# weibohuang0314/pixel_aware_gyro_aided_klt_feature_tracker

Measured on AMD Instinct MI355X. Metric: tracked features/sec (21x21, 3-lvl, 30 iter), higher is better.
Workload: dtype f32 sampling, f64 normal equations; 1 GPU; cfg1_euroc_752x480: 752x480 pair, 1000 keypoints (1000/GPU), gyro-predicted affine init, h=10, L=3, I=30 (synthetic stand-in for BASELINE configs[1]); mode=shard-weak, features_total=1000, features_active=1000, step_mode=graph

## Files before the change

### __graft_entry__.py

```python
from __future__ import annotations

import os
import subprocess
import sys

ROOT = os.path.dirname(os.path.abspath(__file__))
PKG = os.path.join(ROOT, "pixel_aware_gyro_aided_klt_feature_tracker_amd")
CSRC = os.path.join(PKG, "csrc")
HIP_LIB = os.path.join(PKG, "libpagk_hip.so")
HOST_LIB = os.path.join(PKG, "libpagk_tracker.so")

HIPCC_FLAGS = [
    "--offload-arch=gfx950", "-O3", "-std=c++17", "-fPIC", "-shared",
    "-ffp-contract=off", "-fno-fast-math",
    "-Wall", "-Wno-unused-function",
]


def _newer(target: str, sources: list[str]) -> bool:
    if not os.path.exists(target):
        return False
    t = os.path.getmtime(target)
    return all(os.path.getmtime(s) <= t for s in sources)


def _run(cmd: list[str]) -> str:
    r = subprocess.run(cmd, capture_output=True, text=True)
    if r.returncode != 0:
        sys.stderr.write(r.stdout + r.stderr)
        raise RuntimeError("build failed: " + " ".join(cmd))
    return r.stderr


RESOURCES_JSON = os.path.join(PKG, "kernel_resources.json")

RESOURCE_CLAIMS = {
    "k_track_blockILi2ELi25ELi4ELb0ELb0ELb1": (128, 0, 4),
    "k_track_blockILi1ELi25ELi4ELb0ELb0ELb1": (96, 0, 4),
    "k_track_quadILi7ELb1": (128, 44, 4),
    "k_track_blockILi2ELi25ELi4ELb0ELb0ELb0": (128, 20, 4),
    "k_track_blockILi1ELi25ELi4ELb0ELb0ELb0": (128, 6, 4),
    "k_track_quadILi7ELb0": (128, 48, 4),
    "k_track_block_pyrILi2ELi25ELb0": (128, 24, 4),
    "k_track_resume_liveILi2ELi25ELb0": (128, 64, 4),
    "k_track_resumeILi2ELi25ELb0": (128, 64, 4),
    "k_track_resume_liveILi2ELi25ELb1": (128, 48, 4),
    "k_track_resumeILi2ELi25ELb1": (128, 48, 4),
    "k_track_block_pyrILi2ELi25ELb1": (128, 8, 4),
    "k_track_block5ILi2ELi25ELb1": (96, 16, 5),
    "k_rectifyILi1ELb1": (64, 0, 8),
    "k_rectifyILi3ELb1": (64, 0, 8),
    "k_rectifyILi4ELb1": (64, 0, 8),
}


RESOURCE_CLAIMS_ALL_VARIANTS = {
    "k_track_blockILi4ELi25ELi2ELb1ELb0ELb1": (128, 10, 4),
    "k_track_blockILi4ELi25ELi2ELb1ELb0ELb0": (128, 32, 4),
    "k_track_rowsILi7": (128, 64, 4),
}


def _parse_resource_remarks(text: str) -> dict:
    import re
    out, cur = {}, None
    keys = {"VGPRs": "vgprs", "AGPRs": "agprs", "ScratchSize [bytes/lane]": "scratch_bytes_per_lane",
            "Occupancy [waves/SIMD]": "waves_per_simd", "VGPRs Spill": "vgpr_spills", "SGPRs Spill": "sgpr_spills",
            "TotalSGPRs": "sgprs"}
    for line in text.splitlines():
        m = re.search(r"remark:\s+Function Name: (\S+)", line)
        if m:
            cur = out.setdefault(m.group(1), {})
            continue
        m = re.search(r"remark:\s+([A-Za-z \[\]/]+): (\d+)", line)
        if m and cur is not None and m.group(1).strip() in keys:
            cur[keys[m.group(1).strip()]] = int(m.group(2))
    return out


def _parse_resources_from_asm(text: str) -> dict:
    import re
    out, cur, fn = {}, None, None
    keys = {".vgpr_count": "vgprs", ".agpr_count": "agprs", ".private_segment_fixed_size": "scratch_bytes_per_lane",
            ".vgpr_spill_count": "vgpr_spills", ".sgpr_spill_count": "sgpr_spills", ".sgpr_count": "sgprs",
            ".group_segment_fixed_size": "lds_bytes"}
    occ = {}
    for line in text.splitlines():
        m = re.match(r"^(_Z\w+):", line)
        if m:
            fn = m.group(1)
            continue
        m = re.match(r"^; Occupancy: (\d+)", line)
        if m and fn:
            occ[fn] = int(m.group(1))
            continue
        if line.startswith("  - .agpr_count:") or line.startswith("  - .args:"):
            cur = {}
        m = re.match(r"^\s+(?:- )?(\.[a-z_]+):\s+(\S+)\s*$", line)
        if m and cur is not None:
            if m.group(1) == ".name":
                out[m.group(2)] = cur
            elif m.group(1) in keys and m.group(2).isdigit():
                cur[keys[m.group(1)]] = int(m.group(2))
    for k, v in out.items():
        v["waves_per_simd"] = occ.get(k, 0)
        for f in ("vgprs", "agprs", "scratch_bytes_per_lane", "vgpr_spills", "sgpr_spills", "sgprs"):
            v.setdefault(f, 0)
    return {k: v for k, v in out.items() if "vgprs" in v}


def check_resources(res: dict, claims: dict | None = None) -> None:
    bad = []
    for key, (max_vgpr, max_spill, min_occ) in (claims or RESOURCE_CLAIMS).items():
        hits = [v for k, v in res.items() if key in k]
        if not hits:
            bad.append(f"kernel {key} is missing from the code object")
        for v in hits:
            if v["vgprs"] > max_vgpr or v["vgpr_spills"] > max_spill or v["waves_per_simd"] < min_occ:
                bad.append(f"{key}: {v} violates the documented allocation (<= {max_vgpr} VGPRs, <= {max_spill} "
                           f"spilled, >= {min_occ} waves/SIMD)")
    if bad:
        raise RuntimeError("; ".join(bad))


PRIORITY_CLAIMS = {
    "k_track_blockILi2ELi25ELi4ELb0ELb0ELb1": (3, 2, 1, 0),
    "k_track_blockILi2ELi25ELi4ELb0ELb0ELb0": (3, 2, 1, 0),
    "k_track_block5ILi2ELi25ELb1": (3, 2, 0),
}


def check_priorities(asm_text: str, claims: dict | None = None) -> list[str]:
    import re
    body, fn = {}, None
    for line in asm_text.splitlines():
# ... 129 lines not shown
```

### pixel_aware_gyro_aided_klt_feature_tracker_amd/csrc/pagk_hip.hip

```cpp
#include <hip/hip_runtime.h>

#include <algorithm>
#include <array>
#include <cmath>
#include <cstdio>
#include <cstdlib>
#include <cstring>
#include <new>
#include <utility>
#include <vector>

#include "../../include/pagk.h"
#include "pagk_kernels.h"
#include "pagk_layout.h"
#include "pagk_select.h"

using namespace pagk;

namespace {

constexpr int kSlots = 6;
constexpr int kUserSlots = 4;

struct DevBuf {
// ... 21 lines not shown
    int device = 0;
    hipStream_t own_stream = nullptr;
    hipStream_t stream = nullptr;
    FrameSlot slots[kSlots];
    enum Buf {
        FEAT,
        SCORE,
        FIT,
        FITIO,
        HAND,
        HANDIO,
        DET,
        FAST,
        RECT_ENTRIES,
        RECT_STAGE,
        QUAD_WS,
        SUSP,
        LV,
        kBufs
    };
    DevBuf buf[kBufs];
    int fit_n = 0, fit_iters = 0;
    int rect_w = 0, rect_h = 0, rect_wp = 0;
    void *queue = nullptr;
    int quad_capacity[PAGK_MAX_HALF_PATCH + 1] = {};
    int rows_capacity[PAGK_MAX_HALF_PATCH + 1] = {};
    int rows_waves_cap = 0;
    int *susp_count_dev = nullptr;
    struct BatchDesc {
        void *host = nullptr, *dev = nullptr;
        hipEvent_t used = nullptr;
        bool recorded = false;
    };
    static constexpr int kBatchRing = 6, kBatchPerCapture = 4, kBatchMaxStreams = 64;
    BatchDesc batch_ring[kBatchRing];
    int batch_turn = 0;
    bool batch_seen = false;
    std::vector<BatchDesc> cap_batch;
    int cap_batch_used = 0;
    hipEvent_t ev_batch = nullptr;
    int *lv_error = nullptr;
    int *lv_error_dev = nullptr;
    hipStream_t aux_stream = nullptr;
    hipEvent_t ev_fork = nullptr, ev_join = nullptr;
    int susp_lone = 1;
    int finisher_wgs = 16;
    int finisher_polls = 20000;
    int level_polls = 300000;
    int quad_budget = -1;
    int cus = 0;
    bool capturing = false;
    static constexpr int kGraphs = 8;
    hipGraph_t graphs[kGraphs] = {};
    hipGraphExec_t graph_execs[kGraphs] = {};
    struct GraphSeg {
        enum Kind { GRAPH, FINISHER, JOIN } kind = GRAPH;
        hipGraph_t g = nullptr;
        hipGraphExec_t ex = nullptr;
        const void *fn = nullptr;
        TrackArgs args;
        int grid = 0;
        size_t lds = 0;
    };
    std::vector<GraphSeg> pre_segs[kGraphs];
    std::vector<BatchDesc> graph_batch[kGraphs];
    std::vector<GraphSeg> cap_segs;
    hipEvent_t ev_trk[2] = {}, ev_pyr[2] = {};
    bool trk_timed = false, pyr_timed = false;
    int kernel = 0;
    bool last_handover = false;
    int concurrency = 1;
    int last_variant = -1;
    int mfma_min_features = 0x7fffffff;
    int wave_min_features = 6000;
    int quad_min_features = 7000;
    int block5_min_features = 2500;
    int prio_k = 4;
    unsigned long long *prio_stats = nullptr;
    bool block5_window = true;
    int levels_min_features = 6000;
    int levels_shift = 0;
    bool levels_shared = false;
    bool unfused_pyramid = false;
    char err[256] = {0};
};

namespace {

#define HIPCHK(ctx, call)                                                                              \
    do {                                                                                               \
        hipError_t e_ = (call);                                                                        \
        if (e_ != hipSuccess) {                                                                        \
            snprintf((ctx)->err, sizeof((ctx)->err), "%s:%d %s -> %s", __FILE__, __LINE__, #call,     \
                     hipGetErrorString(e_));                                                           \
            return e_ == hipErrorOutOfMemory ? PAGK_E_NOMEM : PAGK_E_HIP;                              \
        }                                                                                              \
    } while (0)

#define NOT_WHILE_CAPTURING(ctx, what)                                                                 \
    do {                                                                                               \
        if ((ctx)->capturing) {                                                                        \
            snprintf((ctx)->err, sizeof((ctx)->err), "%s is not capturable: use the *_device entry points between pagk_graph_begin and pagk_graph_end", what); \
            return PAGK_E_ARG;                                                                         \
        }                                                                                              \
    } while (0)

int level_dims(int w, int h, int L, int *lw, int *lh)
{
    lw[0] = w;
    lh[0] = h;
    for (int l = 1; l < L; l++) {
        lw[l] = (int)(lw[l - 1] * 0.5);
        lh[l] = (int)(lh[l - 1] * 0.5);
        if (lw[l] < 1 || lh[l] < 1) return PAGK_E_ARG;
    }
    return PAGK_OK;
}

bool in_capture(pagk_ctx *ctx)
{
    if (ctx->capturing) return true;
    hipStreamCaptureStatus st = hipStreamCaptureStatusNone;
    return hipStreamIsCapturing(ctx->stream, &st) != hipSuccess || st != hipStreamCaptureStatusNone;
}

int no_live_graphs(pagk_ctx *ctx, const char *what, const char *hint)
{
    for (int k = 0; k < pagk_ctx::kGraphs; k++)
        if (ctx->graph_execs[k]) {
            snprintf(ctx->err, sizeof(ctx->err), "%s would have to grow while graph %d of this context is alive (its nodes hold the old "
                     "pointers): destroy the graph first, or %s", what, k, hint);
            return PAGK_E_ARG;
        }
    return PAGK_OK;
}

enum GrowPolicy {
    GROW_FREELY = 0,
    NOT_IN_CAPTURE = 1,
    NOT_UNDER_GRAPH = 2,
    NOT_IN_CAPTURE_NOR_UNDER_GRAPH = NOT_IN_CAPTURE | NOT_UNDER_GRAPH,
};

int release(pagk_ctx *ctx, DevBuf &b)
{
    if (b.ptr) HIPCHK(ctx, hipFree(b.ptr));
    if (b.host) HIPCHK(ctx, hipHostFree(b.host));
    b.ptr = b.host = nullptr;
    b.bytes = 0;
    return PAGK_OK;
}

int reserve(pagk_ctx *ctx, DevBuf &b, size_t bytes, GrowPolicy policy, const char *what, const char *hint = "")
{
    if (bytes <= b.bytes) return PAGK_OK;
    if ((policy & NOT_IN_CAPTURE) && in_capture(ctx)) {
        snprintf(ctx->err, sizeof(ctx->err), "%s would have to grow inside a graph capture: %s", what, hint);
        return PAGK_E_ARG;
    }
    int rc = (policy & NOT_UNDER_GRAPH) ? no_live_graphs(ctx, what, hint) : PAGK_OK;
    if (rc || (rc = release(ctx, b))) return rc;
    HIPCHK(ctx, hipMalloc(&b.ptr, bytes));
    if (b.mirrored) HIPCHK(ctx, hipHostMalloc(&b.host, bytes, hipHostMallocDefault));
    b.bytes = bytes;
    return PAGK_OK;
}
// ... 66 lines not shown
            return nullptr;
        }
        return &lead->cap_batch[lead->cap_batch_used++];
    }
    pagk_ctx::BatchDesc *desc = &lead->batch_ring[lead->batch_turn];
    lead->batch_turn = (lead->batch_turn + 1) % pagk_ctx::kBatchRing;
    if (!desc->dev) {
        if ((*rc = batch_desc_alloc(lead, *desc)) != PAGK_OK) {
            batch_desc_free(*desc);
            return nullptr;
        }
    } else if (desc->recorded) {
        if (hipEventSynchronize(desc->used) != hipSuccess) {
            snprintf(lead->err, sizeof(lead->err), "hipEventSynchronize of a batch descriptor's last user failed");
            *rc = PAGK_E_HIP;
            return nullptr;
        }
    }
    lead->batch_seen = true;
    return desc;
}
int batch_desc_used(pagk_ctx *lead, pagk_ctx::BatchDesc *desc)
{
    if (in_capture(lead)) return PAGK_OK;
    HIPCHK(lead, hipEventRecord(desc->used, lead->stream));
    desc->recorded = true;
    return PAGK_OK;
}

int slot_alloc(pagk_ctx *ctx, FrameSlot &s, const int *lw, const int *lh, int L, GrowPolicy policy)
{
    size_t sizes[2 * kMaxLevels];
    for (int l = 0; l < L; l++) {
        sizes[l] = (size_t)lw[l] * lh[l];
        sizes[L + l] = sizes[l] * 4;
    }
    const Layout<2 * kMaxLevels> lay(sizes, 2 * L);
    int rc = reserve(ctx, s.block, lay.total, policy, "the frame slot", "run the same calls once before pagk_graph_begin");
    if (rc) return rc;
    for (int l = 0; l < L; l++) {
        s.u8[l] = lay.at<uint8_t>(s.block.ptr, l);
        s.quad[l] = lay.at<uint32_t>(s.block.ptr, L + l);
    }
    s.w = lw[0];
    s.h = lh[0];
    s.L = L;
    return PAGK_OK;
}

int slot_reserve(pagk_ctx *ctx, FrameSlot &s, int w, int h, int L)
{
    int lw[kMaxLevels], lh[kMaxLevels];
    int rc = level_dims(w, h, L, lw, lh);
    return rc ? rc : slot_alloc(ctx, s, lw, lh, L, NOT_IN_CAPTURE);
}

int make_pyr_args(const FrameSlot &s, const uint8_t *src0, int64_t pitch0, int wrap0, PyrArgs *out)
{
    int lw[kMaxLevels], lh[kMaxLevels];
    level_dims(s.w, s.h, s.L, lw, lh);
    PyrArgs pa;
    memset(&pa, 0, sizeof pa);
    pa.src = src0;
    pa.pitch = pitch0;
    pa.wrap0 = wrap0;
    pa.n_levels = s.L;
    int nb = 0;
    for (int l = 0; l < 4; l++) {
        pa.first_block[l] = nb;
        if (l < s.L) {
            pa.cols[l] = lw[l];
            pa.rows[l] = lh[l];
            pa.u8[l] = s.u8[l];
            pa.quad[l] = s.quad[l];
            nb += (lw[l] * lh[l] + 255) / 256;
        }
    }
    pa.first_block[4] = nb;
    for (int l = s.L; l < 4; l++) pa.first_block[l] = nb;
    *out = pa;
    return nb;
}

bool pyramid_fusable(const FrameSlot &s)
{
    int lw[kMaxLevels], lh[kMaxLevels];
    level_dims(s.w, s.h, s.L, lw, lh);
    bool all_even = s.L <= 4;
    for (int l = 0; l + 1 < s.L; l++) all_even = all_even && !(lw[l] & 1) && !(lh[l] & 1);
    return all_even;
}

int slot_build(pagk_ctx *ctx, FrameSlot &s, const uint8_t *src0, int64_t pitch0, int wrap0)
{
    s.pad0 = wrap0 ? 0 : 2;
    s.img0 = src0, s.pitch0 = pitch0;
    int lw[kMaxLevels], lh[kMaxLevels];
    level_dims(s.w, s.h, s.L, lw, lh);
    dim3 blk(32, 8);
    if (ctx->ev_pyr[0] && !in_capture(ctx)) HIPCHK(ctx, hipEventRecord(ctx->ev_pyr[0], ctx->stream));
    bool all_even = true;
    for (int l = 0; l + 1 < s.L; l++) all_even = all_even && !(lw[l] & 1) && !(lh[l] & 1);
    if (s.L <= 4 && !ctx->unfused_pyramid && all_even) {
        PyrArgs pa;
        const int nb = make_pyr_args(s, src0, pitch0, wrap0, &pa);
        hipLaunchKernelGGL(k_pyramid_fused, dim3(nb), dim3(256), 0, ctx->stream, pa);
        HIPCHK(ctx, hipGetLastError());
        if (ctx->ev_pyr[1] && !in_capture(ctx)) HIPCHK(ctx, hipEventRecord(ctx->ev_pyr[1], ctx->stream));
        if (!in_capture(ctx)) ctx->pyr_timed = true;
        s.wrap0 = wrap0;
        s.valid = true;
        return PAGK_OK;
    }
    const uint8_t *src = src0;
    int64_t pitch = pitch0;
    for (int l = 0; l < s.L; l++) {
        if (l > 0) {
            dim3 grd((lw[l] + 31) / 32, (lh[l] + 7) / 8);
            if (!(lw[l - 1] & 1) && !(lh[l - 1] & 1))
                hipLaunchKernelGGL(k_pyr_down, grd, blk, 0, ctx->stream, src, pitch, lw[l], lh[l], s.u8[l]);
            else
                hipLaunchKernelGGL(k_pyr_down_linear, grd, blk, 0, ctx->stream, src, pitch, lw[l - 1], lh[l - 1], lw[l],
                                   lh[l], 1. / ((double)lw[l] / lw[l - 1]), 1. / ((double)lh[l] / lh[l - 1]), s.u8[l]);
            src = s.u8[l];
            pitch = lw[l];
        }
        dim3 grd((lw[l] + 31) / 32, (lh[l] + 7) / 8);
        hipLaunchKernelGGL(k_build_quads, grd, blk, 0, ctx->stream, src, pitch, lw[l], lh[l], l == 0 ? wrap0 : 1,
                           s.quad[l]);
    }
    HIPCHK(ctx, hipGetLastError());
    if (ctx->ev_pyr[1] && !in_capture(ctx)) HIPCHK(ctx, hipEventRecord(ctx->ev_pyr[1], ctx->stream));
    if (!in_capture(ctx)) ctx->pyr_timed = true;
    s.wrap0 = wrap0;
    s.valid = true;
    return PAGK_OK;
}

int check_params(const pagk_params *p)
{
    if (!p) return PAGK_E_ARG;
    if (p->half_patch < 1 || p->half_patch > PAGK_MAX_HALF_PATCH) return PAGK_E_ARG;
    if (p->iterations < 0 || p->pyramids < 1 || p->pyramids > PAGK_MAX_PYRAMIDS) return PAGK_E_ARG;
    if (p->inverse) return PAGK_E_UNSUPPORTED;
    if (p->solver_variant & ~(SV_LOWER_SEQ | SV_UPPER_TREE | SV_NORM_SEQ | SV_LLT_RECIP | SV_PIVOT_TREE)) return PAGK_E_ARG;
    return PAGK_OK;
}

void fill_level(DevLevel &d, const FrameSlot &s, int l)
{
    int w = s.w, h = s.h;
    for (int k = 0; k < l; k++) {
        w = (int)(w * 0.5);
        h = (int)(h * 0.5);
    }
    d.quad = s.quad[l];
    d.cols = w;
    d.rows = h;
    d.fcols = (float)w;
    d.frows = (float)h;
    d.fcols_m1 = (float)(w - 1);
    d.frows_m1 = (float)(h - 1);
}

int lv_check(pagk_ctx *ctx)
{
    if (ctx->lv_error && *static_cast<volatile int *>(ctx->lv_error) != 0) {
        *static_cast<volatile int *>(ctx->lv_error) = 0;
        snprintf(ctx->err, sizeof(ctx->err), "a wave of a tracking launch gave up waiting (for the level above, or for the other chain wave's sums)");
        return PAGK_E_HIP;
    }
    return PAGK_OK;
}

using TrackFn = void (*)(TrackArgs);
struct TrackKernels {
    TrackFn block[2] = {}, block5 = nullptr;
    void (*block_pyr[2])(TrackArgs, PyrArgs) = {};
    TrackFn resume[2] = {}, resume_live[2] = {};
    TrackFn wave[2] = {};
    TrackFn quad[2] = {}, levels[2] = {}, batch[2] = {};
    TrackFn relaxed = nullptr;
    TrackFn mfma[2] = {}, rows = nullptr;
};

template <int H>
constexpr TrackKernels track_kernels()
{
    constexpr PatchShape s = patch_shape(H);
// ... 416 lines not shown
        case PAGK_E_ARG: return "invalid argument";
        case PAGK_E_HIP: return "HIP runtime error";
        case PAGK_E_NOMEM: return "out of memory";
        case PAGK_E_UNSUPPORTED: return "unsupported mode";
        case PAGK_E_NODEVICE: return "no HIP device";
        case PAGK_E_NCCL: return "RCCL error";
        case PAGK_E_CAPACITY: return "output capacity too small";
        default: return "unknown error";
    }
}

const char *pagk_last_error(const pagk_ctx *ctx) { return ctx ? ctx->err : ""; }

void pagk_params_default(pagk_params *p)
{
    if (!p) return;
    memset(p, 0, sizeof *p);
    p->half_patch = 5;
    p->iterations = 10;
    p->pyramids = 3;
    p->has_gyro_predict_initial = 1;
    p->inverse = 0;
    p->consider_illumination = 1;
    p->consider_affine = 1;
    p->regularization_penalty = 0;
    p->calculate_ncc = 0;
    p->lambda = 1.0f;
    p->alpha = 0.5f;
    p->max_distance = 25;
    p->inv_log_max_dist = 0.0f;
    p->fx = p->fy = 1.0f;
    p->n_dist_coef = 4;
}

float pagk_inv_log_max_dist(float alpha, int32_t max_distance)
{
    float arg = alpha * (float)max_distance + 1;
    float lg = std::log(arg);
    return (float)(1.0 / (double)lg);
}

int pagk_create(pagk_ctx **out, int device)
{
    if (!out) return PAGK_E_ARG;
    *out = nullptr;
    int ndev = 0;
    if (hipGetDeviceCount(&ndev) != hipSuccess || ndev <= 0) return PAGK_E_NODEVICE;
    if (device < 0 || device >= ndev) return PAGK_E_ARG;
    pagk_ctx *ctx = new (std::nothrow) pagk_ctx();
    if (!ctx) return PAGK_E_NOMEM;
    ctx->device = device;
    if (hipSetDevice(device) != hipSuccess || hipStreamCreateWithFlags(&ctx->own_stream, hipStreamNonBlocking) != hipSuccess) {
        delete ctx;
        return PAGK_E_HIP;
    }
    ctx->stream = ctx->own_stream;
    ctx->buf[pagk_ctx::FEAT].mirrored = true;
    if (hipDeviceGetAttribute(&ctx->cus, hipDeviceAttributeMultiprocessorCount, device) != hipSuccess) ctx->cus = 0;
    if (hipMalloc(&ctx->queue, 256) != hipSuccess) {
        pagk_destroy(ctx);
        return PAGK_E_NOMEM;
    }
    {
        void *hp = nullptr;
        void *dp = nullptr;
        if (hipHostMalloc(&hp, 64, hipHostMallocMapped) == hipSuccess) {
            memset(hp, 0, 64);
            if (hipHostGetDevicePointer(&dp, hp, 0) == hipSuccess && dp) {
                ctx->lv_error = static_cast<int *>(hp);
                ctx->lv_error_dev = static_cast<int *>(dp);
            } else {
                (void)hipHostFree(hp);
            }
        }
    }
    if (ctx->cus > 0 && ctx->cus != 256) {
        auto scaled = [&](int v) { return v >= 0x7fffffff / 2 ? v : (int)((long long)v * ctx->cus / 256); };
        ctx->wave_min_features = scaled(ctx->wave_min_features);
        ctx->quad_min_features = scaled(ctx->quad_min_features);
        ctx->levels_min_features = scaled(ctx->levels_min_features);
        ctx->block5_min_features = scaled(ctx->block5_min_features);
    }
    ctx->unfused_pyramid = getenv("PAGK_UNFUSED_PYRAMID") != nullptr;
    if (getenv("PAGK_MFMA_MIN")) ctx->mfma_min_features = atoi(getenv("PAGK_MFMA_MIN"));
    if (getenv("PAGK_WAVE_MIN")) ctx->wave_min_features = atoi(getenv("PAGK_WAVE_MIN"));
    if (getenv("PAGK_QUAD_MIN")) ctx->quad_min_features = atoi(getenv("PAGK_QUAD_MIN"));
    if (getenv("PAGK_BLOCK5_MIN")) ctx->block5_min_features = atoi(getenv("PAGK_BLOCK5_MIN")), ctx->block5_window = false;
    if (getenv("PAGK_LEVELS_MIN")) ctx->levels_min_features = atoi(getenv("PAGK_LEVELS_MIN"));
    if (getenv("PAGK_PRIO_K") && strcmp(getenv("PAGK_PRIO_K"), "auto") == 0) {
        struct { unsigned long long st[2]; int k, pad; } seed = {{3500ull, 1000ull}, ctx->prio_k, 0};
        if (hipMalloc(reinterpret_cast<void **>(&ctx->prio_stats), sizeof seed) != hipSuccess ||
            hipMemcpy(ctx->prio_stats, &seed, sizeof seed, hipMemcpyHostToDevice) != hipSuccess) {
            if (ctx->prio_stats) (void)hipFree(ctx->prio_stats);
            ctx->prio_stats = nullptr;
            (void)hipGetLastError();
        }
    } else if (getenv("PAGK_PRIO_K")) {
        ctx->prio_k = atoi(getenv("PAGK_PRIO_K")) < 0 ? 0 : atoi(getenv("PAGK_PRIO_K"));
    }
    if (getenv("PAGK_LEVELS_XCD_SHIFT")) ctx->levels_shift = atoi(getenv("PAGK_LEVELS_XCD_SHIFT")) & 7;
    if (getenv("PAGK_LEVELS_SHARED")) ctx->levels_shared = atoi(getenv("PAGK_LEVELS_SHARED")) != 0;
    if (getenv("PAGK_QUAD_BUDGET")) ctx->quad_budget = atoi(getenv("PAGK_QUAD_BUDGET"));
    if (getenv("PAGK_ROWS_WAVES")) ctx->rows_waves_cap = atoi(getenv("PAGK_ROWS_WAVES"));
    if (getenv("PAGK_FINISHER_WGS")) ctx->finisher_wgs = atoi(getenv("PAGK_FINISHER_WGS"));
    if (getenv("PAGK_SUSPEND_LONE")) ctx->susp_lone = atoi(getenv("PAGK_SUSPEND_LONE"));
    if (getenv("PAGK_FINISHER_POLLS")) ctx->finisher_polls = atoi(getenv("PAGK_FINISHER_POLLS"));
    if (getenv("PAGK_LEVEL_POLLS")) ctx->level_polls = atoi(getenv("PAGK_LEVEL_POLLS"));
    if (hipStreamCreateWithFlags(&ctx->aux_stream, hipStreamNonBlocking) != hipSuccess ||
        hipEventCreateWithFlags(&ctx->ev_fork, hipEventDisableTiming) != hipSuccess ||
        hipEventCreateWithFlags(&ctx->ev_join, hipEventDisableTiming) != hipSuccess ||
        hipEventCreateWithFlags(&ctx->ev_batch, hipEventDisableTiming) != hipSuccess) {
        pagk_destroy(ctx);
        return PAGK_E_HIP;
    }
    for (int k = 0; k < 2; k++) {
        if (hipEventCreate(&ctx->ev_trk[k]) != hipSuccess || hipEventCreate(&ctx->ev_pyr[k]) != hipSuccess) {
            pagk_destroy(ctx);
            return PAGK_E_HIP;
        }
    }
    *out = ctx;
    return PAGK_OK;
}

void pagk_destroy(pagk_ctx *ctx)
{
    if (!ctx) return;
    (void)hipSetDevice(ctx->device);
    if (ctx->own_stream) (void)hipStreamSynchronize(ctx->own_stream);
    if (ctx->aux_stream) {
        (void)hipStreamSynchronize(ctx->aux_stream);
        (void)hipStreamDestroy(ctx->aux_stream);
    }
    if (ctx->ev_fork) (void)hipEventDestroy(ctx->ev_fork);
    if (ctx->ev_join) (void)hipEventDestroy(ctx->ev_join);
    for (int k = 0; k < pagk_ctx::kGraphs; k++) {
        if (ctx->graph_execs[k]) {
            (void)hipGraphExecDestroy(ctx->graph_execs[k]);
            (void)hipGraphDestroy(ctx->graphs[k]);
        }
        destroy_segs(ctx->pre_segs[k]);
    }
    destroy_segs(ctx->cap_segs);
    for (auto &s : ctx->slots) (void)release(ctx, s.block);
    for (auto &b : ctx->buf) (void)release(ctx, b);
    if (ctx->queue) (void)hipFree(ctx->queue);
    if (ctx->prio_stats) (void)hipFree(ctx->prio_stats);
    for (auto &d : ctx->batch_ring) batch_desc_free(d);
    batch_desc_free(ctx->cap_batch);
    for (int k = 0; k < pagk_ctx::kGraphs; k++) batch_desc_free(ctx->graph_batch[k]);
    if (ctx->ev_batch) (void)hipEventDestroy(ctx->ev_batch);
    if (ctx->lv_error) (void)hipHostFree(ctx->lv_error);
    for (int k = 0; k < 2; k++) {
        if (ctx->ev_trk[k]) (void)hipEventDestroy(ctx->ev_trk[k]);
        if (ctx->ev_pyr[k]) (void)hipEventDestroy(ctx->ev_pyr[k]);
    }
    if (ctx->own_stream) (void)hipStreamDestroy(ctx->own_stream);
    delete ctx;
}

int pagk_set_stream(pagk_ctx *ctx, void *hip_stream)
{
    if (!ctx) return PAGK_E_ARG;
    ctx->stream = hip_stream ? static_cast<hipStream_t>(hip_stream) : ctx->own_stream;
    return PAGK_OK;
}
// ... 103 lines not shown
static int frame_upload_any(pagk_ctx *ctx, int32_t slot, const pagk_image *img, int32_t pyramids)
{
    if (!ctx || slot < 0 || slot >= kSlots || pyramids < 1 || pyramids > PAGK_MAX_PYRAMIDS) return PAGK_E_ARG;
    int rc = check_image(img);
    if (rc) return rc;
    HIPCHK(ctx, hipSetDevice(ctx->device));
    FrameSlot &s = ctx->slots[slot];
    s.valid = false;
    if ((rc = slot_reserve(ctx, s, img->width, img->height, pyramids))) return rc;
    if ((rc = upload_level0(ctx, s, img))) return rc;
    rc = slot_build(ctx, s, s.u8[0], s.w, img->step == img->width);
    s.pad0 = (int)(img->step - img->width > 2 ? 2 : img->step - img->width);
    return rc;
}

int pagk_frame_set_device(pagk_ctx *ctx, int32_t slot, const void *d_data, int32_t width, int32_t height,
                          int64_t step, int32_t pyramids)
{
    if (!ctx || slot < 0 || slot >= kUserSlots || pyramids < 1 || pyramids > PAGK_MAX_PYRAMIDS) return PAGK_E_ARG;
    if (!d_data || width < 1 || height < 1 || step < width) return PAGK_E_ARG;
    if (width >= (1 << 24) || height >= (1 << 24) || (int64_t)width * height >= (1ll << 31)) return PAGK_E_ARG;
    HIPCHK(ctx, hipSetDevice(ctx->device));
    FrameSlot &s = ctx->slots[slot];
    s.valid = false;
    int rc = slot_reserve(ctx, s, width, height, pyramids);
    if (rc) return rc;
    rc = slot_build(ctx, s, static_cast<const uint8_t *>(d_data), step, step == width);
    s.pad0 = (int)(step - width > 2 ? 2 : step - width);
    return rc;
}

int pagk_frame_set_device_batch(pagk_ctx *const *ctxs, int32_t k, const int32_t *slot, const void *const *d_data,
                                const int32_t *width, const int32_t *height, const int64_t *step, int32_t pyramids)
{
    if (!ctxs || k < 1 || k > pagk_ctx::kBatchMaxStreams || !slot || !d_data || !width || !height || !step) return PAGK_E_ARG;
    if (pyramids < 1 || pyramids > PAGK_MAX_PYRAMIDS) return PAGK_E_ARG;
    for (int j = 0; j < k; j++) {
        if (!ctxs[j] || slot[j] < 0 || slot[j] >= kUserSlots || !d_data[j] || width[j] < 1 || height[j] < 1 || step[j] < width[j]) return PAGK_E_ARG;
        if (width[j] >= (1 << 24) || height[j] >= (1 << 24) || (int64_t)width[j] * height[j] >= (1ll << 31)) return PAGK_E_ARG;
        for (int i = 0; i < j; i++)
            if (ctxs[i] == ctxs[j] && slot[i] == slot[j]) return PAGK_E_ARG;
    }
    pagk_ctx *lead = ctxs[0];
    for (int j = 1; j < k; j++)
        if (ctxs[j]->device != lead->device) {
            snprintf(lead->err, sizeof(lead->err), "pagk_frame_set_device_batch: context %d lives on device %d, the first on %d", j, ctxs[j]->device, lead->device);
            return PAGK_E_ARG;
        }
    HIPCHK(lead, hipSetDevice(lead->device));
    bool fused = k > 1;
    for (int j = 0; j < k; j++) {
        pagk_ctx *c = ctxs[j];
        FrameSlot &s = c->slots[slot[j]];
        s.valid = false;
        int rc = slot_reserve(c, s, width[j], height[j], pyramids);
        if (rc) {
            if (c != lead) snprintf(lead->err, sizeof(lead->err), "stream %d: %s", j, c->err);
            return rc;
        }
        fused = fused && pyramid_fusable(s) && !c->unfused_pyramid;
    }
    if (!fused) {
        for (int j = 0; j < k; j++) {
            pagk_ctx *c = ctxs[j];
            FrameSlot &s = c->slots[slot[j]];
            int rc = slot_build(c, s, static_cast<const uint8_t *>(d_data[j]), step[j], step[j] == width[j]);
            s.pad0 = (int)(step[j] - width[j] > 2 ? 2 : step[j] - width[j]);
            if (rc) {
                if (c != lead) snprintf(lead->err, sizeof(lead->err), "stream %d: %s", j, c->err);
                return rc;
            }
        }
        return PAGK_OK;
    }
    int rc = PAGK_OK;
    pagk_ctx::BatchDesc *desc = batch_desc_take(lead, &rc);
    if (!desc) return rc;
    PyrBatchEntry *he = static_cast<PyrBatchEntry *>(desc->host);
    int nb = 0;
    for (int j = 0; j < k; j++) {
        FrameSlot &s = ctxs[j]->slots[slot[j]];
        memset(&he[j], 0, sizeof he[j]);
        he[j].block_base = nb;
        nb += make_pyr_args(s, static_cast<const uint8_t *>(d_data[j]), step[j], step[j] == width[j], &he[j].a);
    }
    for (int j = 1; j < k; j++)
        if (ctxs[j]->stream != lead->stream) {
            HIPCHK(lead, hipEventRecord(ctxs[j]->ev_batch, ctxs[j]->stream));
            HIPCHK(lead, hipStreamWaitEvent(lead->stream, ctxs[j]->ev_batch, 0));
        }
    HIPCHK(lead, hipMemcpyAsync(desc->dev, he, (size_t)k * sizeof(PyrBatchEntry), hipMemcpyHostToDevice, lead->stream));
    if (lead->ev_pyr[0] && !in_capture(lead)) HIPCHK(lead, hipEventRecord(lead->ev_pyr[0], lead->stream));
    hipLaunchKernelGGL(k_pyramid_fused_batch, dim3(nb), dim3(256), 0, lead->stream, static_cast<const PyrBatchEntry *>(desc->dev), (int)k);
    HIPCHK(lead, hipGetLastError());
    if (lead->ev_pyr[1] && !in_capture(lead)) HIPCHK(lead, hipEventRecord(lead->ev_pyr[1], lead->stream));
    if (!in_capture(lead)) lead->pyr_timed = true;
    if ((rc = batch_desc_used(lead, desc)) != PAGK_OK) return rc;
    bool others = false;
    for (int j = 1; j < k; j++) others = others || ctxs[j]->stream != lead->stream;
    if (others) {
        HIPCHK(lead, hipEventRecord(lead->ev_batch, lead->stream));
        for (int j = 1; j < k; j++)
            if (ctxs[j]->stream != lead->stream) HIPCHK(lead, hipStreamWaitEvent(ctxs[j]->stream, lead->ev_batch, 0));
    }
    for (int j = 0; j < k; j++) {
        FrameSlot &s = ctxs[j]->slots[slot[j]];
        s.wrap0 = step[j] == width[j];
        s.pad0 = (int)(step[j] - width[j] > 2 ? 2 : step[j] - width[j]);
        s.img0 = static_cast<const uint8_t *>(d_data[j]), s.pitch0 = step[j];
        s.valid = true;
    }
    return PAGK_OK;
}

void pagk_rectify_params_default(pagk_rectify_params *p)
{
    if (!p) return;
    p->channels = 1;
    p->gray_weight[0] = 4899, p->gray_weight[1] = 9617, p->gray_weight[2] = 1868;
    p->gray_shift = 14;
}

int pagk_rectify_params_check(const pagk_rectify_params *p)
{
    if (!p) return PAGK_E_ARG;
    if (p->channels != 1 && p->channels != 3 && p->channels != 4) return PAGK_E_ARG;
    if (p->channels == 1) return PAGK_OK;
    if (p->gray_shift < 1 || p->gray_shift > 15) return PAGK_E_ARG;
    int64_t sum = 0;
    for (int k = 0; k < 3; k++) {
        if (p->gray_weight[k] < 0) return PAGK_E_ARG;
        sum += p->gray_weight[k];
    }
    return sum == (int64_t)1 << p->gray_shift ? PAGK_OK : PAGK_E_ARG;
}

int pagk_undistort_maps(double fx, double fy, double cx, double cy, const double *dist_coef, int32_t n_dist_coef,
                        double new_fx, double new_fy, double new_cx, double new_cy, int32_t width, int32_t height,
                        float *map_x, float *map_y)
{
    if (!map_x || !map_y || width < 1 || height < 1 || (n_dist_coef != 0 && n_dist_coef != 4 && n_dist_coef != 5)) return PAGK_E_ARG;
    if (n_dist_coef > 0 && !dist_coef) return PAGK_E_ARG;
    if (!std::isfinite(new_fx) || !std::isfinite(new_fy) || new_fx == 0.0 || new_fy == 0.0) return PAGK_E_ARG;
    const double k1 = n_dist_coef >= 4 ? dist_coef[0] : 0.0, k2 = n_dist_coef >= 4 ? dist_coef[1] : 0.0;
    const double p1 = n_dist_coef >= 4 ? dist_coef[2] : 0.0, p2 = n_dist_coef >= 4 ? dist_coef[3] : 0.0;
    const double k3 = n_dist_coef >= 5 ? dist_coef[4] : 0.0;
    for (int32_t r = 0; r < height; r++)
        for (int32_t c = 0; c < width; c++) {
            const double x = ((double)c - new_cx) / new_fx, y = ((double)r - new_cy) / new_fy;
            const double x2 = x * x, y2 = y * y, r2 = x2 + y2, xy2 = (2.0 * x) * y;
            const double kr = 1.0 + ((k3 * r2 + k2) * r2 + k1) * r2;
            const double xd = (x * kr + p1 * xy2) + p2 * (r2 + 2.0 * x2);
            const double yd = (y * kr + p1 * (r2 + 2.0 * y2)) + p2 * xy2;
            map_x[(size_t)r * width + c] = (float)(fx * xd + cx);
            map_y[(size_t)r * width + c] = (float)(fy * yd + cy);
        }
    return PAGK_OK;
}

namespace {

bool rect_fixed(float m, int32_t *s)
{
    const float p = m * 32.0f;
    if (!(std::fabs(p) < 2147483648.0f)) return false;
    *s = (int32_t)std::nearbyintf(p);
    return true;
}

inline int32_t sat_i16(int32_t v) { return v < -32768 ? -32768 : (v > 32767 ? 32767 : v); }

int rect_check_src(pagk_ctx *ctx, const pagk_rectify_params *params, int32_t sw, int32_t sh, int64_t sstep, const char *what)
{
    if (pagk_rectify_params_check(params) != PAGK_OK) {
        snprintf(ctx->err, sizeof(ctx->err), "%s: channels must be 1, 3 or 4; for 3 and 4 the gray weights must be non-negative and sum to 1 << gray_shift, 1 <= gray_shift <= 15", what);
        return PAGK_E_ARG;
// ... 1880 lines not shown
```

### pixel_aware_gyro_aided_klt_feature_tracker_amd/csrc/pagk_kernels.h

```cpp
#pragma once
#include <type_traits>
#include "pagk_device.h"
#include "pagk_chain_asm.h"
#include "pagk_prio.h"

namespace pagk {

__global__ void k_pyr_down(const uint8_t *__restrict__ src, int64_t pitch, int dw, int dh,
                           uint8_t *__restrict__ dst)
{
    int x = blockIdx.x * blockDim.x + threadIdx.x;
    int y = blockIdx.y * blockDim.y + threadIdx.y;
    if (x >= dw || y >= dh) return;
    const uint8_t *r0 = src + (int64_t)(2 * y) * pitch + 2 * x;
    const uint8_t *r1 = r0 + pitch;
    dst[(int64_t)y * dw + x] = (uint8_t)((r0[0] + r0[1] + r1[0] + r1[1] + 2) >> 2);
}

__global__ void k_pyr_down_linear(const uint8_t *__restrict__ src, int64_t pitch, int w, int h, int dw, int dh,
                                  double scale_x, double scale_y, uint8_t *__restrict__ dst)
{
    const int dx = blockIdx.x * blockDim.x + threadIdx.x;
    const int dy = blockIdx.y * blockDim.y + threadIdx.y;
    if (dx >= dw || dy >= dh) return;
    float fy = (float)(((double)dy + 0.5) * scale_y - 0.5);
    int sy = (int)floorf(fy);
    fy -= (float)sy;
    const int b0 = __float2int_rn((1.f - fy) * 2048.f), b1 = __float2int_rn(fy * 2048.f);
    const int y0 = sy < 0 ? 0 : (sy < h ? sy : h - 1);
    const int y1 = sy + 1 < 0 ? 0 : (sy + 1 < h ? sy + 1 : h - 1);
    float fx = (float)(((double)dx + 0.5) * scale_x - 0.5);
    int sx = (int)floorf(fx);
    fx -= (float)sx;
    bool single = false;
    if (sx < 0) fx = 0.f, sx = 0;
    if (sx + 1 >= w) {
        single = true;
        if (sx >= w - 1) fx = 0.f, sx = w - 1;
    }
    const int a0 = __float2int_rn((1.f - fx) * 2048.f), a1 = __float2int_rn(fx * 2048.f);
    const uint8_t *r0 = src + (int64_t)y0 * pitch, *r1 = src + (int64_t)y1 * pitch;
    int S0, S1;
    if (single) {
        S0 = (int)r0[sx] * 2048;
        S1 = (int)r1[sx] * 2048;
    } else {
        S0 = (int)r0[sx] * a0 + (int)r0[sx + 1] * a1;
        S1 = (int)r1[sx] * a0 + (int)r1[sx + 1] * a1;
    }
    dst[(int64_t)dy * dw + dx] = (uint8_t)((((b0 * (S0 >> 4)) >> 16) + ((b1 * (S1 >> 4)) >> 16) + 2) >> 2);
}

__global__ void k_build_quads(const uint8_t *__restrict__ src, int64_t pitch, int cols, int rows, int wrap,
                              uint32_t *__restrict__ quad)
{
    int c = blockIdx.x * blockDim.x + threadIdx.x;
    int r = blockIdx.y * blockDim.y + threadIdx.y;
    if (c >= cols || r >= rows) return;
    auto px = [&](int rr, int cc) -> uint32_t {
        if (cc >= cols) {
            if (!wrap) return 0u;
            cc -= cols;
            rr += 1;
        }
        return rr < rows ? (uint32_t)src[(int64_t)rr * pitch + cc] : 0u;
    };
    uint32_t d0 = px(r, c), d1 = px(r, c + 1), d2 = px(r + 1, c), d3 = px(r + 1, c + 1);
    quad[(int64_t)r * cols + c] = d0 | (d1 << 8) | (d2 << 16) | (d3 << 24);
}

struct PyrArgs {
    const uint8_t *src;
    int64_t pitch;
    int wrap0;
    int n_levels;
    int cols[4], rows[4];
    int first_block[5];
    uint8_t *u8[4];
    uint32_t *quad[4];
};

template <int L>
__device__ __forceinline__ uint32_t pyr_pixel(const uint8_t *__restrict__ src, int64_t pitch, int r, int c)
{
    if constexpr (L == 0) {
        return src[(int64_t)r * pitch + c];
    } else {
        return (pyr_pixel<L - 1>(src, pitch, 2 * r, 2 * c) + pyr_pixel<L - 1>(src, pitch, 2 * r, 2 * c + 1) +
                pyr_pixel<L - 1>(src, pitch, 2 * r + 1, 2 * c) + pyr_pixel<L - 1>(src, pitch, 2 * r + 1, 2 * c + 1) + 2) >> 2;
    }
}

template <int L>
__device__ __forceinline__ void pyr_emit(const PyrArgs &a, int idx)
{
    const int cols = a.cols[L], rows = a.rows[L];
    if (idx >= cols * rows) return;
    const int r = idx / cols, c = idx - r * cols;
    const int wrap = L == 0 ? a.wrap0 : 1;
    auto px = [&](int rr, int cc) -> uint32_t {
        if (cc >= cols) {
            if (!wrap) return 0u;
            cc -= cols;
            rr += 1;
        }
        return rr < rows ? pyr_pixel<L>(a.src, a.pitch, rr, cc) : 0u;
    };
    const uint32_t d0 = px(r, c);
    if constexpr (L >= 2) asm volatile("" ::: "memory");
    const uint32_t d1 = px(r, c + 1);
    if constexpr (L >= 2) asm volatile("" ::: "memory");
    const uint32_t d2 = px(r + 1, c);
    if constexpr (L >= 2) asm volatile("" ::: "memory");
    const uint32_t d3 = px(r + 1, c + 1);
    a.quad[L][idx] = d0 | (d1 << 8) | (d2 << 16) | (d3 << 24);
    if constexpr (L > 0) a.u8[L][idx] = (uint8_t)d0;
}

__device__ __forceinline__ void pyr_block(const PyrArgs &a, int b, int tid)
{
    if (b < a.first_block[1]) {
        pyr_emit<0>(a, (b - a.first_block[0]) * 256 + tid);
    } else if (b < a.first_block[2]) {
        pyr_emit<1>(a, (b - a.first_block[1]) * 256 + tid);
    } else if (b < a.first_block[3]) {
        pyr_emit<2>(a, (b - a.first_block[2]) * 256 + tid);
    } else if (b < a.first_block[4]) {
        pyr_emit<3>(a, (b - a.first_block[3]) * 256 + tid);
    }
}

__global__ void __launch_bounds__(256) k_pyramid_fused(PyrArgs a)
{
    pyr_block(a, (int)blockIdx.x, (int)threadIdx.x);
}

struct PyrBatchEntry {
    PyrArgs a;
    int block_base, pad_;
};
__global__ void __launch_bounds__(256) k_pyramid_fused_batch(const PyrBatchEntry *__restrict__ frames, int k)
{
    int f = 0;
    for (int j = 1; j < k; j++) f = (int)blockIdx.x >= frames[j].block_base ? j : f;
    pyr_block(frames[f].a, (int)blockIdx.x - frames[f].block_base, (int)threadIdx.x);
}

struct PredictArgs {
    int n, width, height;
    int single_homography;
    float half;
    float fx, fy, cx, cy, fx_inv, fy_inv, k1, k2, p1, p2, k3;
    float K[6];
    float r31, r32, r33;
    float inv00, inv01;
    const float *pt_ref;
    float *pt_un, *pt_dist, *affine;
    uint8_t *status;
    const float *d_rot;
    const uint8_t *live;
};

__device__ __forceinline__ void predict_one(const PredictArgs &a, float rx, float ry, float &ux, float &uy, float &dxo,
                                            float &dyo)
{
    float x_normal = (rx - a.cx) * a.fx_inv;
    float y_normal = (ry - a.cy) * a.fy_inv;
    float lambda = a.single_homography ? 1.0f : (float)(1.0 / (double)(a.r31 * x_normal + a.r32 * y_normal + a.r33));
    float pt_x = (a.K[0] * rx + a.K[1] * ry + a.K[2]) * lambda;
    float pt_y = (a.K[3] * rx + a.K[4] * ry + a.K[5]) * lambda;
    float x = (pt_x - a.cx) * a.fx_inv;
    float y = (pt_y - a.cy) * a.fy_inv;
    float r2 = x * x + y * y;
    float r4 = r2 * r2;
    float r6 = r4 * r2;
    float xd = x * (1 + a.k1 * r2 + a.k2 * r4 + a.k3 * r6) + 2 * a.p1 * x * y + a.p2 * (r2 + 2 * x * x);
    float yd = y * (1 + a.k1 * r2 + a.k2 * r4 + a.k3 * r6) + a.p1 * (r2 + 2 * y * y) + 2 * a.p2 * x * y;
    ux = pt_x;
    uy = pt_y;
    dxo = a.fx * xd + a.cx;
    dyo = a.fy * yd + a.cy;
}

__global__ void __launch_bounds__(256) k_gyro_predict(PredictArgs a)
{
    int i = blockIdx.x * blockDim.x + threadIdx.x;
    if (i >= a.n) return;
    if (a.d_rot) {
        for (int k = 0; k < 6; k++) a.K[k] = a.d_rot[k];
        a.r31 = a.d_rot[6], a.r32 = a.d_rot[7], a.r33 = a.d_rot[8];
    }
    a.status[i] = 0;
    a.pt_un[2 * i] = a.pt_un[2 * i + 1] = 0.0f;
    a.pt_dist[2 * i] = a.pt_dist[2 * i + 1] = 0.0f;
    if (a.live && !a.live[i]) return;
    const float rx = a.pt_ref[2 * i], ry = a.pt_ref[2 * i + 1];
    float ux, uy, dxs, dys;
    predict_one(a, rx, ry, ux, uy, dxs, dys);
    const float W = (float)a.width, H = (float)a.height;
    if (ux < 0 || ux >= W || uy < 0 || uy >= H) return;
    if (dxs < 0 || dxs >= W || dys < 0 || dys >= H) return;
    a.pt_un[2 * i] = ux;
    a.pt_un[2 * i + 1] = uy;
    a.pt_dist[2 * i] = dxs;
    a.pt_dist[2 * i + 1] = dys;
    a.status[i] = 1;
    if (!a.affine) return;
    const float cxs[4] = {-a.half, a.half, -a.half, a.half}, cys[4] = {-a.half, -a.half, a.half, a.half};
    double s00 = 0, s01 = 0, s10 = 0, s11 = 0;
#pragma unroll
    for (int j = 0; j < 4; j++) {
        float cux, cuy, t0, t1;
        predict_one(a, rx + cxs[j], ry + cys[j], cux, cuy, t0, t1);
        const float Cx = cux - ux, Cy = cuy - uy;
        s00 += (double)Cx * cxs[j];
        s01 += (double)Cx * cys[j];
        s10 += (double)Cy * cxs[j];
        s11 += (double)Cy * cys[j];
    }
    const float t00 = (float)s00, t01 = (float)s01, t10 = (float)s10, t11 = (float)s11;
    a.affine[4 * i + 0] = (float)((double)t00 * a.inv00 + (double)t01 * a.inv01);
    a.affine[4 * i + 1] = (float)((double)t00 * a.inv01 + (double)t01 * a.inv00);
    a.affine[4 * i + 2] = (float)((double)t10 * a.inv00 + (double)t11 * a.inv01);
    a.affine[4 * i + 3] = (float)((double)t10 * a.inv01 + (double)t11 * a.inv00);
}

struct OutPtrs {
    float *pt_un, *pt_dist;
// ... 864 lines not shown
```

Measured before the change: 12.24 million features/s.

## Build fused pyramid per 4x4 tile with packed-byte downsampling and border pass

Replaces the per-pixel fused pyramid kernel with a tiled one. Each thread loads an 8x8 byte window as 32-bit words and emits level-0 quads plus levels 1 and 2 from registers using SWAR byte averaging, which removes the recursive per-pixel re-reads of the source image. Border pixels and level 3 are handled by separate blocks using an unfenced per-pixel path. The old kernel stays available behind an environment variable. This adds complexity and needs 4-byte alignment for the fast path, and the pyramid is only a small part of the 30-iteration tracking step.

```diff
diff --git a/__graft_entry__.py b/__graft_entry__.py
--- a/__graft_entry__.py
+++ b/__graft_entry__.py
@@ -51,6 +51,10 @@
     "k_rectifyILi1ELb1": (64, 0, 8),
     "k_rectifyILi3ELb1": (64, 0, 8),
     "k_rectifyILi4ELb1": (64, 0, 8),
+    "k_pyramid_fusedE": (80, 0, 6),
+    "k_pyramid_fused_batchE": (80, 0, 6),
+    "k_pyramid_pixelE": (64, 0, 8),
+    "k_pyramid_pixel_batchE": (64, 0, 8),
 }
 
 
diff --git a/pixel_aware_gyro_aided_klt_feature_tracker_amd/csrc/pagk_hip.hip b/pixel_aware_gyro_aided_klt_feature_tracker_amd/csrc/pagk_hip.hip
--- a/pixel_aware_gyro_aided_klt_feature_tracker_amd/csrc/pagk_hip.hip
+++ b/pixel_aware_gyro_aided_klt_feature_tracker_amd/csrc/pagk_hip.hip
@@ -127,6 +127,7 @@
     int levels_shift = 0;
     bool levels_shared = false;
     bool unfused_pyramid = false;
+    bool pyramid_per_pixel = false;
     char err[256] = {0};
 };
 
@@ -359,6 +360,29 @@
     return nb;
 }
 
+int make_pyr_tile_args(const FrameSlot &s, const uint8_t *src0, int64_t pitch0, int wrap0, PyrTileArgs *out)
+{
+    PyrTileArgs t;
+    memset(&t, 0, sizeof t);
+    make_pyr_args(s, src0, pitch0, wrap0, &t.a);
+    const bool aligned = reinterpret_cast<uintptr_t>(src0) % 4 == 0 && pitch0 % 4 == 0;
+    if (aligned && s.w >= 8 && s.h >= 8) {
+        t.fast_i = (s.w - 8) / 4 + 1;
+        t.fast_j = (s.h - 8) / 4 + 1;
+    }
+    int nb = (t.fast_i * t.fast_j + kPyrTileThreads - 1) / kPyrTileThreads;
+    for (int l = 0; l < 4; l++) {
+        t.a.first_block[l] = nb;
+        if (l >= s.L) continue;
+        const int cf = l < 3 ? (4 * t.fast_i) >> l : 0, rf = l < 3 ? (4 * t.fast_j) >> l : 0;
+        const int border = (t.a.cols[l] - cf) * t.a.rows[l] + cf * (t.a.rows[l] - rf);
+        nb += (border + kPyrTileThreads - 1) / kPyrTileThreads;
+    }
+    t.a.first_block[4] = nb;
+    *out = t;
+    return nb;
+}
+
 bool pyramid_fusable(const FrameSlot &s)
 {
     int lw[kMaxLevels], lh[kMaxLevels];
@@ -379,9 +403,15 @@
     bool all_even = true;
     for (int l = 0; l + 1 < s.L; l++) all_even = all_even && !(lw[l] & 1) && !(lh[l] & 1);
     if (s.L <= 4 && !ctx->unfused_pyramid && all_even) {
-        PyrArgs pa;
-        const int nb = make_pyr_args(s, src0, pitch0, wrap0, &pa);
-        hipLaunchKernelGGL(k_pyramid_fused, dim3(nb), dim3(256), 0, ctx->stream, pa);
+        if (ctx->pyramid_per_pixel) {
+            PyrArgs pa;
+            const int nb = make_pyr_args(s, src0, pitch0, wrap0, &pa);
+            hipLaunchKernelGGL(k_pyramid_pixel, dim3(nb), dim3(256), 0, ctx->stream, pa);
+        } else {
+            PyrTileArgs ta;
+            const int nb = make_pyr_tile_args(s, src0, pitch0, wrap0, &ta);
+            hipLaunchKernelGGL(k_pyramid_fused, dim3(nb), dim3(kPyrTileThreads), 0, ctx->stream, ta);
+        }
         HIPCHK(ctx, hipGetLastError());
         if (ctx->ev_pyr[1] && !in_capture(ctx)) HIPCHK(ctx, hipEventRecord(ctx->ev_pyr[1], ctx->stream));
         if (!in_capture(ctx)) ctx->pyr_timed = true;
@@ -964,6 +994,7 @@
         ctx->block5_min_features = scaled(ctx->block5_min_features);
     }
     ctx->unfused_pyramid = getenv("PAGK_UNFUSED_PYRAMID") != nullptr;
+    ctx->pyramid_per_pixel = getenv("PAGK_PYRAMID_PER_PIXEL") != nullptr;
     if (getenv("PAGK_MFMA_MIN")) ctx->mfma_min_features = atoi(getenv("PAGK_MFMA_MIN"));
     if (getenv("PAGK_WAVE_MIN")) ctx->wave_min_features = atoi(getenv("PAGK_WAVE_MIN"));
     if (getenv("PAGK_QUAD_MIN")) ctx->quad_min_features = atoi(getenv("PAGK_QUAD_MIN"));
@@ -1233,7 +1264,10 @@
         FrameSlot &s = ctxs[j]->slots[slot[j]];
         memset(&he[j], 0, sizeof he[j]);
         he[j].block_base = nb;
-        nb += make_pyr_args(s, static_cast<const uint8_t *>(d_data[j]), step[j], step[j] == width[j], &he[j].a);
+        if (lead->pyramid_per_pixel)
+            nb += make_pyr_args(s, static_cast<const uint8_t *>(d_data[j]), step[j], step[j] == width[j], &he[j].t.a);
+        else
+            nb += make_pyr_tile_args(s, static_cast<const uint8_t *>(d_data[j]), step[j], step[j] == width[j], &he[j].t);
     }
     for (int j = 1; j < k; j++)
         if (ctxs[j]->stream != lead->stream) {
@@ -1242,7 +1276,10 @@
         }
     HIPCHK(lead, hipMemcpyAsync(desc->dev, he, (size_t)k * sizeof(PyrBatchEntry), hipMemcpyHostToDevice, lead->stream));
     if (lead->ev_pyr[0] && !in_capture(lead)) HIPCHK(lead, hipEventRecord(lead->ev_pyr[0], lead->stream));
-    hipLaunchKernelGGL(k_pyramid_fused_batch, dim3(nb), dim3(256), 0, lead->stream, static_cast<const PyrBatchEntry *>(desc->dev), (int)k);
+    if (lead->pyramid_per_pixel)
+        hipLaunchKernelGGL(k_pyramid_pixel_batch, dim3(nb), dim3(256), 0, lead->stream, static_cast<const PyrBatchEntry *>(desc->dev), (int)k);
+    else
+        hipLaunchKernelGGL(k_pyramid_fused_batch, dim3(nb), dim3(kPyrTileThreads), 0, lead->stream, static_cast<const PyrBatchEntry *>(desc->dev), (int)k);
     HIPCHK(lead, hipGetLastError());
     if (lead->ev_pyr[1] && !in_capture(lead)) HIPCHK(lead, hipEventRecord(lead->ev_pyr[1], lead->stream));
     if (!in_capture(lead)) lead->pyr_timed = true;
diff --git a/pixel_aware_gyro_aided_klt_feature_tracker_amd/csrc/pagk_kernels.h b/pixel_aware_gyro_aided_klt_feature_tracker_amd/csrc/pagk_kernels.h
--- a/pixel_aware_gyro_aided_klt_feature_tracker_amd/csrc/pagk_kernels.h
+++ b/pixel_aware_gyro_aided_klt_feature_tracker_amd/csrc/pagk_kernels.h
@@ -91,7 +91,7 @@
     }
 }
 
-template <int L>
+template <int L, bool FENCED = true>
 __device__ __forceinline__ void pyr_emit(const PyrArgs &a, int idx)
 {
     const int cols = a.cols[L], rows = a.rows[L];
@@ -99,19 +99,26 @@
     const int r = idx / cols, c = idx - r * cols;
     const int wrap = L == 0 ? a.wrap0 : 1;
     auto px = [&](int rr, int cc) -> uint32_t {
+        bool in = true;
         if (cc >= cols) {
-            if (!wrap) return 0u;
+            in = wrap != 0;
             cc -= cols;
             rr += 1;
         }
-        return rr < rows ? pyr_pixel<L>(a.src, a.pitch, rr, cc) : 0u;
+        in = in && rr < rows;
+        if constexpr (FENCED) {
+            return in ? pyr_pixel<L>(a.src, a.pitch, rr, cc) : 0u;
+        } else {
+            const uint32_t v = pyr_pixel<L>(a.src, a.pitch, in ? rr : 0, cc);
+            return in ? v : 0u;
+        }
     };
     const uint32_t d0 = px(r, c);
-    if constexpr (L >= 2) asm volatile("" ::: "memory");
+    if constexpr (FENCED && L >= 2) asm volatile("" ::: "memory");
     const uint32_t d1 = px(r, c + 1);
-    if constexpr (L >= 2) asm volatile("" ::: "memory");
+    if constexpr (FENCED && L >= 2) asm volatile("" ::: "memory");
     const uint32_t d2 = px(r + 1, c);
-    if constexpr (L >= 2) asm volatile("" ::: "memory");
+    if constexpr (FENCED && L >= 2) asm volatile("" ::: "memory");
     const uint32_t d3 = px(r + 1, c + 1);
     a.quad[L][idx] = d0 | (d1 << 8) | (d2 << 16) | (d3 << 24);
     if constexpr (L > 0) a.u8[L][idx] = (uint8_t)d0;
@@ -130,20 +137,135 @@
     }
 }
 
-__global__ void __launch_bounds__(256) k_pyramid_fused(PyrArgs a)
+__global__ void __launch_bounds__(256) k_pyramid_pixel(PyrArgs a)
 {
     pyr_block(a, (int)blockIdx.x, (int)threadIdx.x);
 }
 
+#ifndef PAGK_PYR_TILE_THREADS
+#define PAGK_PYR_TILE_THREADS 64
+#endif
+constexpr int kPyrTileThreads = PAGK_PYR_TILE_THREADS;
+static_assert(kPyrTileThreads == 64 || kPyrTileThreads == 256, "a tile block is one wave or four");
+
+struct PyrTileArgs {
+    PyrArgs a;
+    int fast_i, fast_j;
+};
+
+__device__ __forceinline__ uint32_t pyr_pair_sums(uint32_t w)
+{
+    return (w & 0x00ff00ffu) + ((w >> 8) & 0x00ff00ffu);
+}
+__device__ __forceinline__ uint32_t pyr_down4(uint32_t row0, uint32_t row1)
+{
+    const uint32_t s = ((pyr_pair_sums(row0) + pyr_pair_sums(row1) + 0x00020002u) >> 2) & 0x00ff00ffu;
+    return (s | (s >> 8)) & 0xffffu;
+}
+__device__ __forceinline__ uint32_t pyr_quad(uint32_t lo0, uint32_t hi0, uint32_t lo1, uint32_t hi1, int c)
+{
+    const uint64_t r0 = ((uint64_t)hi0 << 32) | lo0, r1 = ((uint64_t)hi1 << 32) | lo1;
+    return ((uint32_t)(r0 >> (8 * c)) & 0xffffu) | ((uint32_t)(r1 >> (8 * c)) << 16);
+}
+
+__device__ __forceinline__ void pyr_tile(const PyrTileArgs &t, int idx)
+{
+    const PyrArgs &a = t.a;
+    if (idx >= t.fast_i * t.fast_j) return;
+    const int j = idx / t.fast_i, i = idx - j * t.fast_i;
+    const uint8_t *__restrict__ src = a.src + (int64_t)(4 * j) * a.pitch + 4 * i;
+    uint32_t lo[8], hi[8];
+#pragma unroll
+    for (int k = 0; k < 8; k++) {
+        const uint32_t *row = reinterpret_cast<const uint32_t *>(src + (int64_t)k * a.pitch);
+        lo[k] = row[0];
+        hi[k] = row[1];
+    }
+    uint32_t *__restrict__ q0 = a.quad[0] + (4 * j) * a.cols[0] + 4 * i;
+#pragma unroll
+    for (int r = 0; r < 4; r++) {
+#pragma unroll
+        for (int c = 0; c < 4; c++) q0[r * a.cols[0] + c] = pyr_quad(lo[r], hi[r], lo[r + 1], hi[r + 1], c);
+    }
+    if (a.n_levels < 2) return;
+    uint32_t m[4];
+#pragma unroll
+    for (int r = 0; r < 4; r++) m[r] = pyr_down4(lo[2 * r], lo[2 * r + 1]) | (pyr_down4(hi[2 * r], hi[2 * r + 1]) << 16);
+    const int p1 = (2 * j) * a.cols[1] + 2 * i;
+#pragma unroll
+    for (int r = 0; r < 2; r++) {
+#pragma unroll
+        for (int c = 0; c < 2; c++) {
+            a.quad[1][p1 + r * a.cols[1] + c] = pyr_quad(m[r], 0u, m[r + 1], 0u, c);
+            a.u8[1][p1 + r * a.cols[1] + c] = (uint8_t)(m[r] >> (8 * c));
+        }
+    }
+    if (a.n_levels < 3) return;
+    const uint32_t n0 = pyr_down4(m[0], m[1]), n1 = pyr_down4(m[2], m[3]);
+    const int p2 = j * a.cols[2] + i;
+    a.quad[2][p2] = n0 | (n1 << 16);
+    a.u8[2][p2] = (uint8_t)n0;
+}
+
+template <int L>
+__device__ __forceinline__ void pyr_border(const PyrTileArgs &t, int idx)
+{
+    if constexpr (L >= 3) {
+        pyr_emit<L, false>(t.a, idx);
+    } else {
+        const int cols = t.a.cols[L], rows = t.a.rows[L];
+        const int cf = (4 * t.fast_i) >> L, rf = (4 * t.fast_j) >> L;
+        const int wr = cols - cf, n_right = wr * rows;
+        int r, c;
+        if (idx < n_right) {
+            r = idx / wr;
+            c = cf + idx - r * wr;
+        } else {
+            idx -= n_right;
+            if (idx >= cf * (rows - rf)) return;
+            r = idx / cf;
+            c = idx - r * cf;
+            r += rf;
+        }
+        pyr_emit<L, false>(t.a, r * cols + c);
+    }
+}
+
+__device__ __forceinline__ void pyr_tile_block(const PyrTileArgs &t, int b, int tid)
+{
+    if (b < t.a.first_block[0]) {
+        pyr_tile(t, b * kPyrTileThreads + tid);
+    } else if (b < t.a.first_block[1]) {
+        pyr_border<0>(t, (b - t.a.first_block[0]) * kPyrTileThreads + tid);
+    } else if (b < t.a.first_block[2]) {
+        pyr_border<1>(t, (b - t.a.first_block[1]) * kPyrTileThreads + tid);
+    } else if (b < t.a.first_block[3]) {
+        pyr_border<2>(t, (b - t.a.first_block[2]) * kPyrTileThreads + tid);
+    } else if (b < t.a.first_block[4]) {
+        pyr_border<3>(t, (b - t.a.first_block[3]) * kPyrTileThreads + tid);
+    }
+}
+
+__global__ void __launch_bounds__(kPyrTileThreads) k_pyramid_fused(PyrTileArgs t)
+{
+    pyr_tile_block(t, (int)blockIdx.x, (int)threadIdx.x);
+}
+
 struct PyrBatchEntry {
-    PyrArgs a;
+    PyrTileArgs t;
     int block_base, pad_;
 };
-__global__ void __launch_bounds__(256) k_pyramid_fused_batch(const PyrBatchEntry *__restrict__ frames, int k)
+__global__ void __launch_bounds__(kPyrTileThreads) k_pyramid_fused_batch(const PyrBatchEntry *__restrict__ frames, int k)
 {
     int f = 0;
     for (int j = 1; j < k; j++) f = (int)blockIdx.x >= frames[j].block_base ? j : f;
-    pyr_block(frames[f].a, (int)blockIdx.x - frames[f].block_base, (int)threadIdx.x);
+    pyr_tile_block(frames[f].t, (int)blockIdx.x - frames[f].block_base, (int)threadIdx.x);
+}
+__global__ void __launch_bounds__(256) k_pyramid_pixel_batch(const PyrBatchEntry *__restrict__ frames, int k)
+{
+    int f = 0;
+    for (int j = 1; j < k; j++) f = (int)blockIdx.x >= frames[j].block_base ? j : f;
+    pyr_block(frames[f].t.a, (int)blockIdx.x - frames[f].block_base, (int)threadIdx.x);
 }
 
 struct PredictArgs {
```

New measurement: 12.22 million features/s. Within noise of the previous version (-0.2%).
